# lh3/fermi

Measured on AMD Instinct MI355X. Metric: reads/sec through FMD backward-search (unitig overlap discovery), higher is better.
Workload: dtype u64

## Files before the change

### fermi_amd/csrc/fmd_kernel_common.h

```cpp
#pragma once
#include "fmd_internal.h"

#define NONE64 (~0ull)
#define FMD_SZ_MASK 0xffffffffffffull

__device__ __forceinline__ int comp6(int c) { return (c >= 1 && c <= 4) ? 5 - c : c; }

#include "fmd_search.h"

template <class T>
__device__ __forceinline__ T sel6(int c, T a0, T a1, T a2, T a3, T a4, T a5)
{
    T r = a0;
    r = c == 1 ? a1 : r; r = c == 2 ? a2 : r; r = c == 3 ? a3 : r; r = c == 4 ? a4 : r; r = c == 5 ? a5 : r;
    return r;
}

__device__ __forceinline__ void load_entry(const fmd_intv_t *e, uint64_t &x0, uint64_t &x1, uint64_t &sz, uint64_t &info)
{
    const uint4 *q = (const uint4 *)e;
    const uint4 a = q[0], b = q[1];
    x0 = (uint64_t)a.y << 32 | a.x; x1 = (uint64_t)a.w << 32 | a.z;
    sz = (uint64_t)b.y << 32 | b.x; info = (uint64_t)b.w << 32 | b.z;
}
__device__ __forceinline__ void store_entry(fmd_intv_t *e, uint64_t x0, uint64_t x1, uint64_t sz, uint64_t info)
{
    uint4 *q = (uint4 *)e;
    q[0] = make_uint4((uint32_t)x0, (uint32_t)(x0 >> 32), (uint32_t)x1, (uint32_t)(x1 >> 32));
    q[1] = make_uint4((uint32_t)sz, (uint32_t)(sz >> 32), (uint32_t)info, (uint32_t)(info >> 32));
}

#define FMD_CAND_NARROW 0x80000000u
struct FmdCand { uint64_t x0, x1, sz, D, r0; uint32_t depth; bool narrow; };
__device__ __forceinline__ FmdCand cand_decode(const uint4 a, const uint4 b)
{
    FmdCand c;
    c.narrow = (b.w & FMD_CAND_NARROW) != 0;
    c.x1 = (uint64_t)a.w << 32 | a.z;
    if (c.narrow) {
        c.x0 = (uint64_t)(a.y & 0xffu) << 32 | a.x; c.r0 = (uint64_t)((a.y >> 8) & 0xffu) << 32 | b.z; c.depth = a.y >> 16;
        c.sz = b.w & 63u; c.D = (uint64_t)b.y << 32 | b.x;
    } else {
        c.x0 = (uint64_t)a.y << 32 | a.x; c.sz = ((uint64_t)b.y << 32 | b.x) & 0xffffffffffffull; c.depth = b.z; c.D = 0; c.r0 = 0;
    }
    return c;
}
__device__ __forceinline__ void cand_store(fmd_intv_t *e, bool narrow, uint64_t x0, uint64_t x1, uint64_t sz, uint32_t depth, uint64_t D, uint64_t r0)
{
    uint4 *q = (uint4 *)e;
    const uint32_t x0h = (uint32_t)(x0 >> 32);
    q[0] = make_uint4((uint32_t)x0, narrow ? ((x0h & 0xffu) | ((uint32_t)(r0 >> 32) & 0xffu) << 8 | depth << 16) : x0h, (uint32_t)x1, (uint32_t)(x1 >> 32));
    q[1] = make_uint4(narrow ? (uint32_t)D : (uint32_t)sz, narrow ? (uint32_t)(D >> 32) : (uint32_t)(sz >> 32), narrow ? (uint32_t)r0 : depth,
                      narrow ? (FMD_CAND_NARROW | (uint32_t)sz) : 0u);
}

__device__ __forceinline__ uint64_t bits_below(int j) { return j >= 64 ? ~0ull : ((1ull << j) - 1); }

__device__ __forceinline__ uint4 grp_pick(const uint4 *img_k, int t_k, const uint4 *img_l, int t_l, uint32_t blk_k, uint32_t blk_l,
                                          bool has_k, bool has_l, uint32_t blk, uint32_t ch)
{
    const bool in_k = has_k && blk == blk_k, in_l = has_l && blk == blk_l;
    uint4 v = in_k ? img_k[(int)ch ^ t_k] : img_l[(int)ch ^ t_l];
    if (!in_k && !in_l) v = make_uint4(0, 0, 0, 0);
    return v;
}
__device__ __forceinline__ void grp_window(const uint4 *img_k, int t_k, const uint4 *img_l, int t_l, uint32_t blk_k, uint32_t blk_l,
                                           bool has_k, bool has_l, uint32_t blk_p, uint32_t off_p, uint4 &a, uint4 &b, uint4 &c)
{
    uint32_t blk = blk_p, ch = (off_p + 1) >> 5;
    if (ch >= FMD_BLK_CHUNKS) { ch -= FMD_BLK_OWN_CHUNKS; ++blk; }
    a = grp_pick(img_k, t_k, img_l, t_l, blk_k, blk_l, has_k, has_l, blk, ch);
    if (++ch == FMD_BLK_CHUNKS) { ch = FMD_BLK_CHUNKS - FMD_BLK_OWN_CHUNKS; ++blk; }
    b = grp_pick(img_k, t_k, img_l, t_l, blk_k, blk_l, has_k, has_l, blk, ch);
    if (++ch == FMD_BLK_CHUNKS) { ch = FMD_BLK_CHUNKS - FMD_BLK_OWN_CHUNKS; ++blk; }
    c = grp_pick(img_k, t_k, img_l, t_l, blk_k, blk_l, has_k, has_l, blk, ch);
}
__device__ __forceinline__ uint64_t win64(uint32_t w0, uint32_t w1, uint32_t w2, uint32_t sh)
{
    const uint32_t lo = __builtin_amdgcn_alignbit(w1, w0, sh), hi = __builtin_amdgcn_alignbit(w2, w1, sh);
    return (uint64_t)hi << 32 | lo;
}
template <class T>
__device__ __forceinline__ T win_before(T X, T Y, T Z, T cx, T cy, T cz)
{
    return ~(X | Y | Z) | (Z & ~X & (cx | cy)) | (X & Y & (cx ^ cy)) | (Y & ~X & cx & ~cy) | (X & ~Y & ~Z & cx & cz);
}
__device__ __forceinline__ uint64_t range64(uint32_t a, uint32_t b)
{
    return bits_below((int)b) & ~bits_below((int)a);
}


#define FMD_GRP_CLASSES 6
__device__ __host__ __forceinline__ constexpr int fmd_grp_size(int k) { return k == 0 ? 4 : k == 1 ? 8 : k == 2 ? 12 : k == 3 ? 16 : k == 4 ? 21 : 32; }
#define FMD_FAST_CHUNK 16
#define FMD_FAST_MAX_WAVES 8192
#define FMD_LIST_HOLE 0xffffffffu
#define FMD_LIST_RESUME 0x8000u
__device__ __forceinline__ void fmd_resume_encode(uint4 *e, uint64_t x1, uint32_t sz, uint64_t D, uint64_t r0, uint32_t pos, uint32_t round, uint32_t n_nei, uint32_t nei0, uint32_t lf,
                                                  uint32_t cat = 0, uint32_t flags8 = 0)
{
    e[0] = make_uint4((uint32_t)x1, ((uint32_t)(x1 >> 32) & 0xffu) | round << 8 | n_nei << 24, (uint32_t)D, (uint32_t)(D >> 32));
    e[1] = make_uint4((uint32_t)r0, ((uint32_t)(r0 >> 32) & 0xffu) | nei0 << 8, sz | pos << 16, (lf & 0x1ffffu) | cat << 17 | (flags8 & 0xffu) << 22);
}
__device__ __forceinline__ bool fmd_resume_fits(uint32_t round, uint32_t n_nei, uint32_t nei0, uint32_t pos) { return round < 65536u && n_nei < 256u && nei0 < 65536u && pos < 65536u; }
__device__ __forceinline__ void fmd_resume_decode(const uint4 a, const uint4 b, uint64_t &x1, uint32_t &sz, uint64_t &D, uint64_t &r0, uint32_t &pos, uint32_t &round, uint32_t &n_nei,
                                                  uint32_t &nei0, uint32_t &lf, uint32_t &cat, uint32_t &flags8)
{
    x1 = (uint64_t)(a.y & 0xffu) << 32 | a.x; round = (a.y >> 8) & 0xffffu; n_nei = a.y >> 24; D = (uint64_t)a.w << 32 | a.z;
    r0 = (uint64_t)(b.y & 0xffu) << 32 | b.x; nei0 = b.y >> 8; sz = b.z & 0xffffu; pos = b.z >> 16; lf = b.w & 0x1ffffu; cat = (b.w >> 17) & 31u; flags8 = (b.w >> 22) & 0xffu;
}
#define FMD_LANE_CHUNK 64
#define FMD_FAST_RESERVE (2 * FMD_FAST_MAX_WAVES * FMD_LANE_CHUNK)

#define FMD_CLS_CNT_STRIDE 32
#define FMD_CLS_HEADER_U32 640
#define FMD_CLS_LISTS (3 * FMD_GRP_CLASSES + 1)
#define FMD_CLS_SLOW FMD_GRP_CLASSES
static_assert(FMD_CLS_LISTS * FMD_CLS_CNT_STRIDE <= FMD_CLS_HEADER_U32, "one counter line per list");
__host__ __device__ __forceinline__ constexpr int fmd_cls_fast(int k) { return FMD_GRP_CLASSES + 1 + k; }
__host__ __device__ __forceinline__ constexpr int fmd_cls_cnt_off(int c) { return c * FMD_CLS_CNT_STRIDE; }
template <class P>
__host__ __device__ __forceinline__ constexpr P fmd_cls_list(P area, int c, size_t np)
{
    const size_t gl = 2 * np + 2 * (size_t)FMD_FAST_RESERVE;
    const P slow = area + FMD_CLS_HEADER_U32 + gl * FMD_GRP_CLASSES;
    if (c == FMD_CLS_SLOW) return slow;
    return c < FMD_CLS_SLOW ? area + FMD_CLS_HEADER_U32 + gl * c : slow + np + 2 * np * (size_t)(c - FMD_CLS_SLOW - 1);
}
template <class P> __host__ __device__ __forceinline__ constexpr P fmd_cls_late(P area, size_t np) { return fmd_cls_list(area, FMD_CLS_LISTS, np); }
template <class P> __host__ __device__ __forceinline__ constexpr P fmd_cls_fix(P area, size_t np) { return fmd_cls_late(area, np) + np; }
#define FMD_CLS_WORDS_PER_STRAND (6 * FMD_GRP_CLASSES + 3)
#define FMD_CLS_PART_U32 (FMD_CLS_HEADER_U32 + 2 * FMD_GRP_CLASSES * FMD_FAST_RESERVE)
__host__ __device__ __forceinline__ constexpr size_t fmd_cls_part_off(int part, size_t b) { return (size_t)part * FMD_CLS_PART_U32 + b * FMD_CLS_WORDS_PER_STRAND; }
static_assert(fmd_cls_fix<size_t>(0, 1000) + 1000 == fmd_cls_part_off(1, 1000) && fmd_cls_fix<size_t>(0, 1) + 1 == fmd_cls_part_off(1, 1), "a part's lists end where the next part begins");

enum FmdClsWord {
    FMD_CW_COUNT = 0,
    FMD_CW_DEAL = 16,
    FMD_CW_DOWN = 4,
    FMD_CW_DOWN_DEAL = FMD_CW_DOWN + FMD_CW_DEAL,
    FMD_CW_HANDED = 8,
    FMD_CW_HANDED_AT0 = 9,
    FMD_CW_FAST_ROUNDS = 10,
    FMD_CW_FAST_LIVE = 11,
    FMD_CW_FAST_HELD = 12,
    FMD_CW_FAST_ROUNDS2 = 13,
    FMD_CW_LATE = 4,
    FMD_CW_GRP_ROUNDS = 12,
    FMD_CW_GRP_LIVE = 13,
    FMD_CW_GRP_HELD = 14,
    FMD_CW_FIX = 20,
};
template <int... W> constexpr bool fmd_cw_distinct()
{
    const int w[] = {W...};
    for (size_t i = 0; i < sizeof...(W); ++i) {
        if (w[i] < 0 || w[i] >= FMD_CLS_CNT_STRIDE) return false;
        for (size_t j = 0; j < i; ++j) if (w[j] == w[i]) return false;
    }
    return true;
}
static_assert(fmd_cw_distinct<FMD_CW_COUNT, FMD_CW_DEAL>(), "a general list's counter line");
static_assert(fmd_cw_distinct<FMD_CW_COUNT, FMD_CW_DEAL, FMD_CW_DOWN, FMD_CW_DOWN_DEAL, FMD_CW_HANDED, FMD_CW_HANDED_AT0, FMD_CW_FAST_ROUNDS, FMD_CW_FAST_LIVE, FMD_CW_FAST_HELD,
                              FMD_CW_FAST_ROUNDS2>(), "a fast list's counter line");
static_assert(fmd_cw_distinct<FMD_CW_COUNT, FMD_CW_LATE, FMD_CW_GRP_ROUNDS, FMD_CW_GRP_LIVE, FMD_CW_GRP_HELD, FMD_CW_FIX>(), "the slow list's counter line");

struct FmdOvlClasses {
    uint32_t *cnt;
    uint32_t *lst[FMD_GRP_CLASSES];
    uint32_t *lslow;
    uint32_t *fast[2 * FMD_GRP_CLASSES];
};

__device__ __forceinline__ int fmd_ovl_list_of(uint32_t m, uint32_t len, bool w63, bool wnarrow, bool w32, int use_fast, int min_cls)
{
    int c = FMD_CLS_SLOW;
    if (w63 && len < 65535u) {
#pragma unroll
        for (int k = FMD_GRP_CLASSES - 1; k >= 0; --k) if (k >= min_cls && m <= (uint32_t)fmd_grp_size(k)) c = k;
        if (c < FMD_CLS_SLOW && wnarrow && use_fast) c += fmd_cls_fast(w32 ? FMD_GRP_CLASSES : 0);
    }
    return c;
}

#define FMD_WALK_SPLIT 32u
struct FmdWalkPark {
    unsigned long long k, x0, x1, sz;
    uint4 bases;
    uint4 pad;
};
static_assert(sizeof(FmdWalkPark) == 64, "one line per parked strand");
```

### fermi_amd/csrc/fmd_ovlp.hip

```cpp
#include <stdlib.h>
#include <string.h>
#include "fmd_ovlp_internal.h"

struct BatchLayout { size_t srev, listA, listB, cls, total; uint32_t stride_r, cap; };
static BatchLayout batch_layout(size_t n, uint32_t max_len, int min_match)
{
    BatchLayout L;
    const size_t stride_r = align_up((size_t)max_len, 16), cap = fmd_ovlp_list_cap(max_len, min_match);
    L.stride_r = (uint32_t)stride_r; L.cap = (uint32_t)cap;
    size_t o = 0;
    L.srev = o; o += align_up(n * stride_r, 256);
    L.listA = o; o += align_up(n * cap * sizeof(fmd_intv_t), 256);
    L.listB = o; o += align_up(n * cap * sizeof(fmd_intv_t), 256);
    L.cls = o; o += align_up(4 * fmd_cls_part_off(FMD_OVLP_MAX_PARTS, n), 256) + 256;
    L.total = o;
    return L;
}
extern "C" size_t fmd_ovlp_work_bytes(size_t n, uint32_t max_len, int min_match) { return batch_layout(n, max_len, min_match).total; }

struct OvlBatch {
    fmd_dev *h; FmdIndexView ix;
    const uint64_t *ids; int min_match; uint32_t max_len, max_nei, stride_r, cap, seq_stride;
    uint8_t *srev; fmd_intv_t *listA, *listB; uint32_t *cls;
    fmd_ovlp_rec_t *rec; fmd_intv_t *nei; uint8_t *seq;
    const uint32_t *gidx; FmdWalkPark *park;
    const uint32_t *keys;
    void carve(uint8_t *area, size_t n_area)
    {
        const BatchLayout L = batch_layout(n_area, max_len, min_match);
        stride_r = L.stride_r; cap = L.cap;
        srev = area + L.srev; listA = (fmd_intv_t *)(area + L.listA); listB = (fmd_intv_t *)(area + L.listB); cls = (uint32_t *)(area + L.cls);
    }
};

static bool ovl_tail2(const OvlBatch &o)
{
    const char *e = getenv("FMD_WALK_TAIL2");
    return o.gidx && fmd_walk_tail2_fits(o.stride_r, o.seq_stride) && !(e && atoi(e) == 0);
}
static bool ovl_tail2_cls(const OvlBatch &o)
{
    const char *e = getenv("FMD_WALK_CLS");
    return ovl_tail2(o) && !(e && atoi(e) == 0);
}
static int ovl_use_fast(void) { const char *ef = getenv("FMD_OVLP_FAST"); return fmd_nei_fast_available() && !(ef && atoi(ef) == 0); }
static int ovl_grp_down(void) { const char *e = getenv("FMD_GRP_DOWN"); return !(e && atoi(e) == 0); }
static int ovl_walk_phase(void) { const char *e = getenv("FMD_WALK_PHASE"); return !(e && atoi(e) == 0); }
static int ovl_min_cls(void) { const char *e = getenv("FMD_GRP4"); return e && atoi(e) == 0 ? 1 : 0; }

static void ovl_phase_a(const OvlBatch &o, hipStream_t st, size_t b, size_t np, int per_cu)
{
    WalkArgs a;
    a.ix = o.ix; a.n = np; a.min_match = o.min_match; a.stride_r = o.stride_r;
    a.listA = o.listA + b * (size_t)o.cap; a.cap = o.cap;
    uint8_t *srev = o.srev + b * (size_t)o.stride_r;
    if (!o.gidx) {
        a.ids = o.ids + b; a.rec = o.rec + b; a.srev = srev;
        fmd_launch_walk_whole(o.h, st, a, o.max_len, o.seq + b * (size_t)o.seq_stride, o.seq_stride, per_cu, 64);
        return;
    }
    a.rec = o.rec; a.park = o.park; a.gidx = o.gidx + b;
    if (!ovl_tail2(o)) {
        a.srev = srev;
        fmd_launch_walk_tail(o.h, st, a, o.max_len, o.seq, o.seq_stride, per_cu);
        return;
    }
    a.seq_out = o.seq; a.seq_stride = o.seq_stride; a.redo = (uint32_t *)srev;
    if (ovl_tail2_cls(o)) {
        a.cls = o.cls + fmd_cls_part_off(0, b); a.use_fast = ovl_use_fast(); a.min_cls = ovl_min_cls();
    }
    if (o.keys && ovl_walk_phase()) a.keys = o.keys + b;
    fmd_launch_walk_tail2(o.h, st, a, per_cu);
}

static int ovl_phase_b(const OvlBatch &o, hipStream_t st, size_t b, size_t np, int part, int per_cu, int fast_cu)
{
    NeiArgs a;
    a.ix = o.ix; a.n_cu = o.h->n_cu; a.grid = fmd_grid_for(o.h, np); a.np = np; a.min_match = o.min_match;
    a.srev = o.srev + b * (size_t)o.stride_r; a.stride_r = o.stride_r;
    a.listA = o.listA + b * (size_t)o.cap; a.listB = o.listB + b * (size_t)o.cap; a.cap = o.cap;
    a.gidx = o.gidx ? o.gidx + b : nullptr;
    a.rec = a.gidx ? o.rec : o.rec + b;
    a.nei = a.gidx ? o.nei : o.nei + b * (size_t)o.max_nei; a.max_nei = o.max_nei;
    a.seq = a.gidx ? o.seq : o.seq + b * (size_t)o.seq_stride; a.seq_stride = o.seq_stride;
    uint32_t *q2 = fmd_next_queue(o.h, st);
    uint32_t *cls = o.cls + fmd_cls_part_off(part, b);
    fmd_nei_lists_at(a, cls, np);
    const int use_fast = ovl_use_fast();
    if (!(part == 0 && ovl_tail2_cls(o))) {
        FMD_HIP_TRY(hipMemsetAsync(cls, 0, 4 * FMD_CLS_HEADER_U32, st));
        fmd_launch_classify(a, st, use_fast, ovl_min_cls());
    }
    bool side = false;
    FmdSideStream &slow = o.h->slow;
    if (slow.acquire(2)) {
        side = hipEventRecord(slow.ev[0], st) == hipSuccess && hipStreamWaitEvent(slow.stream, slow.ev[0], 0) == hipSuccess;
        if (!side) { (void)hipGetLastError(); slow.release(); }
    }
    {
        hipStream_t ss = side ? slow.stream : st;
        fmd_launch_nei_slow(a, ss, fmd_next_queue(o.h, ss), 0);
    }
    if (use_fast)
        for (int k = 0; k < 2 * FMD_GRP_CLASSES; ++k) {
            const int kg = k % FMD_GRP_CLASSES, wide = k >= FMD_GRP_CLASSES;
            if (fmd_nei_lane_enabled() && fmd_nei_lane_class_ok(kg, wide)) fmd_launch_nei_lane(a, kg, wide, fast_cu, st);
            else fmd_launch_nei_fast(a, kg, wide, fast_cu, st);
        }
    const uint32_t down_cap = ovl_grp_down() && np > 2 * (size_t)FMD_FAST_CHUNK ? (uint32_t)np : 0u;
    for (int k = 0; k < FMD_GRP_CLASSES; ++k) fmd_launch_nei_grp(a, k, per_cu, st, down_cap, 0);
    if (down_cap)
        for (int k = FMD_GRP_CLASSES - 2; k >= 0; --k) fmd_launch_nei_grp(a, k, per_cu, st, down_cap, 1);
    fmd_launch_nei_slow(a, st, q2, 1);
    fmd_launch_nei_fix(a, st, fmd_next_queue(o.h, st));
    if (side) {
        if (hipEventRecord(slow.ev[1], slow.stream) != hipSuccess || hipStreamWaitEvent(st, slow.ev[1], 0) != hipSuccess) { (void)hipGetLastError(); hipStreamSynchronize(slow.stream); }
        slow.release();
    }
    if (getenv("FMD_OVLP_STATS")) {
        uint32_t hs[FMD_CLS_HEADER_U32];
        hipStreamSynchronize(st);
        hipMemcpy(hs, cls, sizeof(hs), hipMemcpyDeviceToHost);
        const auto word = [&hs](int c, int w) { return hs[fmd_cls_cnt_off(c) + w]; };
        uint32_t nf = 0, nb = 0, ng = 0;
        for (int k = 0; k < 2 * FMD_GRP_CLASSES; ++k) { nf += word(fmd_cls_fast(k), FMD_CW_COUNT); nb += word(fmd_cls_fast(k), FMD_CW_HANDED); }
        for (int k = 0; k < FMD_GRP_CLASSES; ++k) ng += word(k, FMD_CW_COUNT);
        fprintf(stderr, "[M::fmd_ovlp] part of %zu strands: %u to the unforked path (%u of them handed on), %u slots of the general group kernels' lists (holes of the hand-over included), %u through the lane-per-strand kernel at once + %u handed back to it, %u fake forks fixed up\n",
                np, nf, nb, ng, word(FMD_CLS_SLOW, FMD_CW_COUNT), word(FMD_CLS_SLOW, FMD_CW_LATE), word(FMD_CLS_SLOW, FMD_CW_FIX));
        uint32_t ne[FMD_GRP_CLASSES];
        for (int k = 0; k < FMD_GRP_CLASSES; ++k) {
            const size_t slots = word(k, FMD_CW_COUNT);
            uint32_t *e = (uint32_t *)malloc(8 * slots + 8);
            ne[k] = 0;
            if (e && hipMemcpy(e, a.cl.lst[k], 8 * slots, hipMemcpyDeviceToHost) == hipSuccess)
                for (size_t i = 0; i < slots; ++i) ne[k] += e[2 * i] != FMD_LIST_HOLE;
            free(e);
        }
        static_assert(FMD_GRP_CLASSES == 6, "one %u per general class");
        fprintf(stderr, "[M::fmd_ovlp] ... of those slots %u %u %u %u %u %u hold a strand (general lists of the group classes, smallest first)\n", ne[0], ne[1], ne[2], ne[3], ne[4], ne[5]);
    }
#ifdef GRP_STATS
    {
        uint32_t hs[FMD_CLS_HEADER_U32];
        hipStreamSynchronize(st);
        hipMemcpy(hs, cls, sizeof(hs), hipMemcpyDeviceToHost);
        const auto word = [&hs](int c, int w) { return hs[fmd_cls_cnt_off(c) + w]; };
        const uint32_t gr = word(FMD_CLS_SLOW, FMD_CW_GRP_ROUNDS), gl = word(FMD_CLS_SLOW, FMD_CW_GRP_LIVE), gh = word(FMD_CLS_SLOW, FMD_CW_GRP_HELD);
        static_assert(FMD_GRP_CLASSES == 6, "one %u per general class");
        fprintf(stderr, "[grp stats] classes %u %u %u %u %u %u slow %u | wave rounds %u, live lanes %u (%.1f %%), lanes of groups holding a strand %u (%.1f %%)\n",
                word(0, FMD_CW_COUNT), word(1, FMD_CW_COUNT), word(2, FMD_CW_COUNT), word(3, FMD_CW_COUNT), word(4, FMD_CW_COUNT), word(5, FMD_CW_COUNT), word(FMD_CLS_SLOW, FMD_CW_COUNT),
                gr, gl, 100.0 * gl / (64.0 * gr), gh, 100.0 * gh / (64.0 * gr));
        for (int k = 0; k < 2 * FMD_GRP_CLASSES; ++k) {
            const int f = fmd_cls_fast(k);
            const uint32_t fr = word(f, FMD_CW_FAST_ROUNDS);
            if (word(f, FMD_CW_COUNT)) fprintf(stderr, "[fast stats] G=%d %s: %u strands, %u handed on (%u) | wave rounds %u (%u with a second base), live lanes %.1f %%, lanes of groups holding a strand %.1f %%\n",
                              fmd_grp_size(k % FMD_GRP_CLASSES), k >= FMD_GRP_CLASSES ? "64-bit" : "32-bit", word(f, FMD_CW_COUNT), word(f, FMD_CW_HANDED), word(f, FMD_CW_HANDED_AT0), fr,
                              word(f, FMD_CW_FAST_ROUNDS2), 100.0 * word(f, FMD_CW_FAST_LIVE) / (64.0 * fr), 100.0 * word(f, FMD_CW_FAST_HELD) / (64.0 * fr));
        }
    }
#endif
    return FMD_OK;
}

static void ovl_pipe_config(size_t n, int &parts, int &walk_cu, int &grp_cu, int &fast_cu)
{
    parts = 1; walk_cu = 8; grp_cu = 8; fast_cu = 8;
    const char *e = getenv("FMD_OVLP_PIPE");
    if (e) {
        int a = 0, b = 0, c = 0, d = 0;
        const int k = sscanf(e, "%d,%d,%d,%d", &a, &b, &c, &d);
        if (k >= 1 && a >= 1) parts = a < FMD_OVLP_MAX_PARTS ? a : FMD_OVLP_MAX_PARTS;
        if (k >= 2 && b >= 1) walk_cu = b;
        if (k >= 3 && c >= 1) grp_cu = c;
        if (k >= 4 && d >= 1) fast_cu = d;
    }
}
extern "C" int fmd_ovlp_dev(fmd_dev_t *h, void *stream_, size_t n, const uint64_t *d_ids, int min_match, uint32_t max_len,
                            uint32_t max_nei, fmd_ovlp_rec_t *d_rec, fmd_intv_t *d_nei, uint8_t *d_seq, uint32_t seq_stride,
                            void *d_work, size_t work_bytes)
{
    if (!h || (n && (!d_ids || !d_rec || !d_nei || !d_seq || !d_work)) || max_len == 0 || max_nei == 0 || min_match < 0) return FMD_E_ARG;
    if (n == 0) return FMD_OK;
    if (n >= 0xffffff00ull || work_bytes < fmd_ovlp_work_bytes(n, max_len, min_match)) return FMD_E_ARG;
    if (fmd_ovlp_list_cap(max_len, min_match) >= 4096) return FMD_E_ARG;
    FMD_HIP_TRY(hipSetDevice(h->device));
    hipStream_t st = (hipStream_t)stream_;
    OvlBatch o;
    o.h = h; o.ix = fmd_view(h);
    o.ids = d_ids; o.min_match = min_match; o.max_len = max_len; o.max_nei = max_nei; o.seq_stride = seq_stride;
    o.carve((uint8_t *)d_work, n);
    o.rec = d_rec; o.nei = d_nei; o.seq = d_seq; o.gidx = nullptr; o.park = nullptr; o.keys = nullptr;

    int parts, walk_cu, grp_cu, fast_cu;
    ovl_pipe_config(n, parts, walk_cu, grp_cu, fast_cu);
    if (parts > 1 && !h->aux.acquire(FMD_OVLP_MAX_PARTS + 1)) parts = 1;
    int rc = FMD_OK;
    if (parts == 1) {
        ovl_phase_a(o, st, 0, n, 0);
        rc = ovl_phase_b(o, st, 0, n, 0, 0, 0);
    } else {
        hipStream_t s2 = h->aux.stream;
        const size_t per = ((n + parts - 1) / parts + 63) & ~(size_t)63;
        int p = 0;
        bool join_ok = true;
        for (size_t b = 0; b < n && rc == FMD_OK; b += per, ++p) {
            const size_t np = n - b < per ? n - b : per;
            const bool last = b + per >= n;
            ovl_phase_a(o, st, b, np, p == 0 ? 0 : walk_cu);
            if (hipEventRecord(h->aux.ev[p], st) != hipSuccess || hipStreamWaitEvent(s2, h->aux.ev[p], 0) != hipSuccess) { join_ok = false; break; }
            rc = ovl_phase_b(o, s2, b, np, p, last ? 0 : grp_cu, last ? 0 : fast_cu);
        }
        if (!join_ok || hipEventRecord(h->aux.ev[FMD_OVLP_MAX_PARTS], s2) != hipSuccess ||
            hipStreamWaitEvent(st, h->aux.ev[FMD_OVLP_MAX_PARTS], 0) != hipSuccess) {
            hipStreamSynchronize(s2);
            if (!join_ok) { fmd_set_hip_error(hipGetLastError(), "overlap batch: event hand-over"); rc = FMD_E_HIP; }
        }
        h->aux.release();
    }
    if (rc != FMD_OK) return rc;
    FMD_CHECK_LAUNCH("overlap kernels");
    return FMD_OK;
}

struct SortedLayout { size_t park, keys_a, keys_b, vals_a, vals_b, tmp, tmp_bytes, batch_area, total; };
static SortedLayout sorted_layout(size_t n, size_t batch, uint32_t max_len, int min_match)
{
    SortedLayout L;
    size_t o = 0;
    L.park = o; o += align_up(n * sizeof(FmdWalkPark), 256);
    L.keys_a = o; o += align_up(n * 4, 256);
    L.keys_b = o; o += align_up(n * 4, 256);
    L.vals_a = o; o += align_up(n * 4, 256);
    L.vals_b = o; o += align_up(n * 4, 256);
    L.tmp_bytes = fmd_park_sort_temp_bytes(n);
    L.tmp = o; o += align_up(L.tmp_bytes, 256);
    L.batch_area = o;
    { const size_t ba = fmd_ovlp_work_bytes(batch, max_len, min_match), ad = align_up(n * 32, 256); o += ba > ad ? ba : ad; }
    L.total = o;
    return L;
}
extern "C" size_t fmd_ovlp_sorted_work_bytes(size_t n, size_t batch, uint32_t max_len, int min_match)
{
    if (batch == 0 || batch > n) batch = n;
    return sorted_layout(n, batch, max_len, min_match).total;
}
static bool sorted_eligible(const fmd_dev *h, size_t n, int min_match, uint32_t max_len)
{
    const char *e = getenv("FMD_OVLP_SORT");
    if (e && atoi(e) == 0) return false;
    return n < 0xffffff00ull && min_match >= (int)FMD_WALK_SPLIT && max_len >= FMD_WALK_SPLIT && h->ptab_d < (int)FMD_WALK_SPLIT;
}

extern "C" int fmd_ovlp_two_pass_ok(const fmd_dev_t *h, size_t n, int min_match, uint32_t max_len)
{
    return h && sorted_eligible(h, n, min_match, max_len) && fmd_ovlp_list_cap(max_len, min_match) < 4096 ? 1 : 0;
}
struct HeadLayout { size_t adm, keys_a, vals_a, tmp, tmp_bytes, total; };
static HeadLayout head_layout(size_t n)
{
    HeadLayout L;
    size_t o = 0;
    L.keys_a = o; o += align_up(n * 4, 256);
    L.vals_a = o; o += align_up(n * 4, 256);
    L.tmp_bytes = fmd_park_sort_temp_bytes(n);
    L.tmp = o; o += align_up(L.tmp_bytes, 256);
    L.adm = o; o += align_up(n * 32, 256);
    L.total = o;
    return L;
}
extern "C" size_t fmd_ovlp_head_work_bytes(size_t n) { return head_layout(n).total; }

extern "C" int fmd_ovlp_head_dev(fmd_dev_t *h, void *stream_, size_t n, const uint64_t *d_ids, int min_match, uint32_t max_len, fmd_ovlp_rec_t *d_rec,
                                 void *d_park, uint32_t *d_keys, uint32_t *d_order, void *d_work, size_t work_bytes)
{
    if (!h || (n && (!d_ids || !d_rec || !d_park || !d_keys || !d_order || !d_work)) || max_len == 0 || min_match < 0) return FMD_E_ARG;
    if (n == 0) return FMD_OK;
    if (!fmd_ovlp_two_pass_ok(h, n, min_match, max_len)) return FMD_E_ARG;
    const HeadLayout L = head_layout(n);
    if (work_bytes < L.total) return FMD_E_ARG;
    FMD_HIP_TRY(hipSetDevice(h->device));
    uint8_t *w = (uint8_t *)d_work;
    const int rc = fmd_ovlp_head(h, (hipStream_t)stream_, n, d_ids, min_match, d_rec, (FmdWalkPark *)d_park, (uint32_t *)(w + L.keys_a), (uint32_t *)(w + L.vals_a),
                            d_keys, d_order, w + L.tmp, L.tmp_bytes, (uint4 *)(w + L.adm));
    if (rc != FMD_OK) return rc;
    FMD_CHECK_LAUNCH("sorted overlap job: head");
    return FMD_OK;
}

static int ovl_tail(fmd_dev *h, hipStream_t st, size_t np, const uint32_t *rows, const uint32_t *keys, FmdWalkPark *park, const uint64_t *d_ids, int min_match, uint32_t max_len, uint32_t max_nei,
                    fmd_ovlp_rec_t *d_rec, fmd_intv_t *d_nei, uint8_t *d_seq, uint32_t seq_stride, uint8_t *area, size_t area_strands)
{
    OvlBatch o;
// ... 214 lines not shown
```

### fermi_amd/csrc/fmd_ovlp_lane.hip

```cpp
#include "fmd_ovlp_internal.h"

#define LANE_CHUNK FMD_LANE_CHUNK

template <typename M> struct LaneW;
template <> struct LaneW<uint32_t> {
    static constexpr uint32_t MAXW = 31;
    static __device__ __forceinline__ uint32_t below(uint32_t n) { return (1u << n) - 1u; }
    static __device__ __forceinline__ uint32_t popc(uint32_t v) { return (uint32_t)__popc(v); }
    static __device__ __forceinline__ int top(uint32_t v) { return 31 - __clz((int)v); }
};
template <> struct LaneW<uint64_t> {
    static constexpr uint32_t MAXW = 63;
    static __device__ __forceinline__ uint64_t below(uint32_t n) { return (1ull << n) - 1ull; }
    static __device__ __forceinline__ uint32_t popc(uint64_t v) { return (uint32_t)__popcll(v); }
    static __device__ __forceinline__ int top(uint64_t v) { return 63 - __clzll((long long)v); }
};

#define LC_PACK(r0, d, sz, pos) ((uint32_t)((r0) >> 32) & 0xffu) | (uint32_t)(d) << 8 | (uint32_t)(sz) << 14 | (uint32_t)(pos) << 20
#define LC_D(p) (((p) >> 8) & 63u)
#define LC_SZ(p) (((p) >> 14) & 63u)
#define LC_POS(p) ((p) >> 20)
#define LC_R0(p, lo) ((uint64_t)((p) & 0xffu) << 32 | (lo))
#define LANE_MAX_LEN 4095u


__device__ __forceinline__ void lane_flush_bases(uint8_t *seq_out, uint32_t seq_stride, uint32_t gs, uint32_t ori_l, uint32_t from, uint32_t to, uint64_t eb)
{
    uint8_t *row = seq_out + gs * (size_t)seq_stride;
    uint32_t p = ori_l + from, e = ori_l + to;
    if (e > seq_stride) e = seq_stride;
    while (p < e && (p & 3u)) { row[p] = (uint8_t)((eb & 3u) + 1u); eb >>= 2; ++p; }
    while (p + 4 <= e) {
        const uint32_t b = (uint32_t)eb & 0xffu;
        *(uint32_t *)(row + p) = ((b & 3u) | (b & 0xcu) << 6 | (b & 0x30u) << 12 | (b & 0xc0u) << 18) + 0x01010101u;
        eb >>= 8; p += 4;
    }
    while (p < e) { row[p] = (uint8_t)((eb & 3u) + 1u); eb >>= 2; ++p; }
}

#ifndef FMD_LANE_LB
#define FMD_LANE_LB 2
#endif

template <int G, typename M>
__global__ __launch_bounds__(64, FMD_LANE_LB) void k_ovl_nei_lane(FmdIndexView ix, const uint32_t *__restrict__ list, const uint32_t *__restrict__ list_n,
                                                                uint32_t cap, const fmd_intv_t *__restrict__ listA, fmd_intv_t *__restrict__ listB, fmd_ovlp_rec_t *__restrict__ rec,
                                                                fmd_intv_t *__restrict__ nei_out, uint32_t max_nei, uint8_t *__restrict__ seq_out, uint32_t seq_stride,
                                                                uint32_t *__restrict__ gen_list, uint32_t *__restrict__ gen_n, uint32_t *__restrict__ bail_n,
                                                                const uint32_t *__restrict__ gidx, uint32_t *__restrict__ queue, uint32_t tk_chunk, uint32_t slow_min, uint32_t adm_min)
{
    using W = LaneW<M>;
    constexpr bool WIDE = sizeof(M) == 8;
    __shared__ uint4 fmd_lds[WIDE ? FMD_WAVE_LDS_U4 : FMD_SLOT_U4];
    uint4 *lds = fmd_lds;
    const int lane = fmd_lane();
    const uint32_t N = *list_n;
    if (N == 0) return;
    FmdTickets tk;
    fmd_tickets_init(tk, queue, tk_chunk, N);

    bool active = false;
    uint32_t sid = 0, gs = 0, meta = 0, n_nei = 0, lf = 0, nei0 = 0, szw = 1, round = 0, am = 0;
    uint64_t X1 = 1;
    uint64_t eb = 0;
    uint32_t eb0 = 0;
    __shared__ uint4 cand[G * 64];
    uint4 *mc = cand + lane;
#define CD(e) (WIDE ? (M)((uint64_t)(e).y << 32 | (e).x) : (M)(e).x)
    uint32_t m_lane = 0;
    uint32_t res_cur = 0, res_end = 0, n_handed = 0;
    int hand = 0;
    bool slow = false;
    M sX = 0, sY = 0, sZ = 0;
    uint64_t sR0 = 0, sR1 = 0, sR2 = 0, sR3 = 0, sR4 = 0;
    int scs = 0;
    int st = 0;
    bool adm_bad = false;
    constexpr int HALVES = G > 8 ? 2 : 1, RAWN = (G + HALVES - 1) / HALVES;
    bool drained = false;

    for (;;) {
        {
            const uint64_t hm = __ballot(hand != 0);
            if (hm) {
                uint32_t meta_out = meta;
                if (hand == 2) {
                    const uint32_t mp = (uint32_t)__popc(am);
                    if (mp <= cap && fmd_resume_fits(round, n_nei, nei0, 0u)) {
                        for (uint32_t j = 0; j < m_lane; ++j)
                            if ((am >> j) & 1u) {
                                const uint4 e = mc[j * 64];
                                fmd_resume_encode((uint4 *)(listB + sid * (size_t)cap + __popc(am & ((1u << j) - 1u))), X1 + LC_D(e.w), LC_SZ(e.w), (uint64_t)CD(e),
                                                  LC_R0(e.w, e.z), LC_POS(e.w), round, n_nei, nei0, lf);
                            }
                        meta_out = mp | FMD_LIST_RESUME | (meta & 0xffff0000u);
                    }
                }
                const uint32_t n = (uint32_t)__popcll(hm), room = res_end - res_cur;
                uint32_t base = 0;
                if (room < n) {
                    if (lane == 0) { base = atomicAdd(gen_n, (uint32_t)LANE_CHUNK); atomicAdd(bail_n, n_handed); }
                    n_handed = 0;
                    base = (uint32_t)__builtin_amdgcn_readfirstlane((int)base);
                    gen_list[2 * (size_t)(base + lane)] = FMD_LIST_HOLE; gen_list[2 * (size_t)(base + lane) + 1] = 0;
                    asm volatile("s_waitcnt vmcnt(0)" ::: "memory");
                }
                if (hand) {
                    const uint32_t q = (uint32_t)fmd_below(hm), k = q < room ? res_cur + q : base + (q - room);
                    gen_list[2 * (size_t)k] = sid; gen_list[2 * (size_t)k + 1] = meta_out;
                    am = 0;
                }
                if (room < n) { res_cur = base + (n - room); res_end = base + LANE_CHUNK; }
                else res_cur += n;
                n_handed += n;
                hand = 0;
            }
        }
        uint4 raw[2 * RAWN];
        uint32_t l0 = 0, l1 = 0, g_in = 0;
        const uint64_t adm_wait_m = __ballot(st >= 2), adm_act_m = __ballot(active);
        const bool ld2 = st >= 2 && ((uint32_t)__popcll(adm_wait_m) >= adm_min || adm_act_m == 0);
        const uint32_t adm_m = meta & 0xffffu, adm_h0 = HALVES == 2 ? adm_m / 2 : 0u;
        const uint32_t adm_base = st == 2 ? adm_h0 : 0u, adm_cnt = st == 2 ? adm_m - adm_h0 : adm_h0;
        if (ld2) {
            const uint4 *q0 = (const uint4 *)(listA + sid * (size_t)cap + (cap - adm_m) + adm_base);
#pragma unroll
            for (int t = 0; t < RAWN; ++t) if ((uint32_t)t < adm_cnt) { raw[2 * t] = q0[2 * t]; raw[2 * t + 1] = q0[2 * t + 1]; }
            if (st == 2) g_in = gidx ? gidx[sid] : sid;
        }
        bool ld1 = false;
        {
            const bool want = st == 0 && !active && !drained && hand == 0;
            const size_t p = fmd_tickets_take(tk, queue, want, N);
            if (want && (p == (size_t)-1 || p >= N)) drained = true;
            else if (want) { l0 = list[2 * p]; l1 = list[2 * p + 1]; ld1 = true; }
        }
        const bool go = active && !slow;
        if (__ballot(go) == 0) fmd_fetch_wait();
        else {
            uint32_t bke, oke;
            fmd_split(X1 - 1, bke, oke);
            const uint4 *img_k, *img_l;
            int t_k, t_l;
            uint32_t ble = bke;
            bool sep = false;
            if (WIDE) {
                const FmdRank2 r = fmd_wave_rank2_fetch(ix, lds, go ? X1 - 1 : NONE64, go ? X1 - 1 + szw : NONE64);
                img_k = r.bk; img_l = r.bl; t_k = r.t; t_l = r.tl; ble = r.blk_l; sep = go && ble != bke;
            } else {
                fmd_fetch_slot<0>(ix, lds, bke, go);
                fmd_fetch_wait();
                img_k = img_l = lds + fmd_lds_base(lane, 0); t_k = t_l = fmd_chunk_xor(lane);
            }
            M X, Y, Z;
            {
                uint4 a, b, c;
                grp_window(img_k, t_k, img_l, t_l, bke, ble, true, sep, bke, oke, a, b, c);
                const uint32_t sh = (uint32_t)X1 & 31;
                if (WIDE) { X = (M)win64(a.x, b.x, c.x, sh); Y = (M)win64(a.y, b.y, c.y, sh); Z = (M)win64(a.z, b.z, c.z, sh); }
                else { X = (M)__builtin_amdgcn_alignbit(b.x, a.x, sh); Y = (M)__builtin_amdgcn_alignbit(b.y, a.y, sh); Z = (M)__builtin_amdgcn_alignbit(b.z, a.z, sh); }
            }
            const M mw = W::below(szw);
            const M any = (X | Y | Z) & mw, xa = X & any, ya = Y & any, za = Z & any;
            const M ends = ~(X | Y | Z) & mw;
            int cs = (xa ? 1 : 0) | (ya ? 2 : 0) | (za ? 4 : 0);
            const bool mixed = go && ((xa && xa != any) || (ya && ya != any) || (za && za != any) || cs > 4);
            uint64_t R[6] = {0, 0, 0, 0, 0, 0};
            if (__ballot(mixed)) { if (mixed) fmd_block_rank6<false>(img_k, t_k, oke + 1, R, bke); }
            if (!mixed) { uint64_t rz; const uint64_t rc = fmd_block_rank1z(img_k, t_k, oke + 1, cs, bke, rz); R[0] = rz; R[1] = R[2] = R[3] = R[4] = rc; }
            if (go) {
                if (!mixed && ends == 0) {
                    if (!(lf & 0x10000u)) lf = round + 1;
                    eb |= (uint64_t)(uint32_t)(4 - cs) << (2 * (round - eb0));
                    ++round;
                    if (round - eb0 == 32) { lane_flush_bases(seq_out, seq_stride, gs, meta >> 16, eb0, round, eb); eb = 0; eb0 = round; }
                    X1 = (cs == 1 ? ix.cnt[1] : cs == 2 ? ix.cnt[2] : cs == 3 ? ix.cnt[3] : ix.cnt[4]) + R[1];
                } else { slow = true; sX = X; sY = Y; sZ = Z; sR0 = R[0]; sR1 = R[1]; sR2 = R[2]; sR3 = R[3]; sR4 = R[4]; scs = cs | (mixed ? 8 : 0); }
            }
        }
        {
            const uint64_t sm = __ballot(slow);
            if (sm && ((uint32_t)__popcll(sm) >= slow_min || __ballot(active && !slow) == 0)) {
                if (slow) {
                    const M X = sX, Y = sY, Z = sZ;
                    int cs = scs & 7;
                    const bool mixed = (scs & 8) != 0;
                    const M mw = W::below(szw), any = (X | Y | Z) & mw, ends = ~(X | Y | Z) & mw;
                    const M m1 = X & ~Y & ~Z & mw, m2 = ~X & Y & ~Z & mw, m3 = X & Y & ~Z & mw, m4 = ~X & ~Y & Z & mw;
                    bool bail = false;
                    if (mixed) {
                        const M m5 = X & ~Y & Z & mw;
                        uint32_t u = 0;
                        for (uint32_t j = 0; j < m_lane; ++j) {
                            if ((am >> j) & 1u) {
                                const uint4 e = mc[j * 64];
                                const uint32_t d = LC_D(e.w), sz = LC_SZ(e.w);
                                const M mine = W::below(sz) << d;
                                const uint32_t nS = W::popc(ends & mine);
                                const uint32_t s1 = W::popc(m1 & mine), s2 = W::popc(m2 & mine), s3 = W::popc(m3 & mine), s4 = W::popc(m4 & mine), s5 = W::popc(m5 & mine);
                                const uint32_t o4 = nS, o3 = o4 + s4, o2 = o3 + s3, o1_ = o2 + s2, o5 = o1_ + s1;
                                const M D = CD(e);
                                if ((D >> o1_) & W::below(s1)) u |= 2u;
                                if ((D >> o2) & W::below(s2)) u |= 4u;
                                if ((D >> o3) & W::below(s3)) u |= 8u;
                                if ((D >> o4) & W::below(s4)) u |= 16u;
                                if ((D >> o5) & W::below(s5)) u |= 32u;
                            }
                        }
                        bail = __popc(u) >= 2 || (u & 32u);
                        cs = u ? __ffs((int)u) - 1 : 0;
                        if (cs > 4) cs = 0;
                    }
                    const uint64_t Rz = sR0, Rc = cs == 1 ? sR1 : cs == 2 ? sR2 : cs == 3 ? sR3 : cs == 4 ? sR4 : sR0;
                    const M Cw = !mixed ? any : cs == 1 ? m1 : cs == 2 ? m2 : cs == 3 ? m3 : cs == 4 ? m4 : (M)0;
                    slow = false;
                    const uint32_t ori_l = meta >> 16;
                    if (bail) { hand = 2; active = false; lane_flush_bases(seq_out, seq_stride, gs, ori_l, eb0, round, eb); }
                    else {
                    uint32_t nei_m = 0, child_m = 0;
                    for (uint32_t j = 0; j < m_lane; ++j) {
                        if ((am >> j) & 1u) {
                            const uint4 e = mc[j * 64];
                            const uint32_t d = LC_D(e.w), sz = LC_SZ(e.w);
                            const M mine = W::below(sz) << d, D = CD(e);
                            const uint32_t nS = W::popc(ends & mine);
                            uint32_t nc, coff;
                            if (mixed) {
                                const uint32_t s1 = W::popc(m1 & mine), s2 = W::popc(m2 & mine), s3 = W::popc(m3 & mine), s4 = W::popc(m4 & mine);
                                const uint32_t o4 = nS, o3 = o4 + s4, o2 = o3 + s3, o1_ = o2 + s2;
                                nc = cs == 1 ? s1 : cs == 2 ? s2 : cs == 3 ? s3 : cs == 4 ? s4 : 0u;
                                coff = cs == 1 ? o1_ : cs == 2 ? o2 : cs == 3 ? o3 : o4;
                            } else { nc = W::popc(any & mine); coff = sz - nc; }
                            if (round > 0 && nS == sz && D == W::below(sz)) nei_m |= 1u << j;
                            if ((D >> coff) & W::below(nc)) child_m |= 1u << j;
                        }
                    }
                    if (!(lf & 0x10000u)) lf = child_m ? round + 1 : (FMD_LFORK_ALL | 0x10000u);
                    const int f = nei_m ? __ffs((int)nei_m) - 1 : 32;
                    const uint32_t keep_m = f >= 32 ? child_m : child_m & ((1u << f) - 1u);
                    if (nei_m) {
                        const uint4 e = mc[f * 64];
                        const uint32_t d = LC_D(e.w), sz = LC_SZ(e.w), pos = LC_POS(e.w);
                        if (n_nei == 0) nei0 = ori_l - pos;
                        if (n_nei < max_nei)
                            store_entry(nei_out + gs * (size_t)max_nei + n_nei, LC_R0(e.w, e.z), ix.cnt[0] + Rz + W::popc(ends & W::below(d)), (uint64_t)sz, (uint64_t)(ori_l - pos));
                        ++n_nei;
                    }
                    if (n_nei > max_nei) {
                        rec[gs].flags |= FMD_OVLP_F_OVERFLOW;
                        active = false; am = 0;
                    } else if (keep_m) {
                        eb |= (uint64_t)(uint32_t)(4 - cs) << (2 * (round - eb0));
                        ++round;
                        if (round - eb0 == 32) { lane_flush_bases(seq_out, seq_stride, gs, ori_l, eb0, round, eb); eb = 0; eb0 = round; }
                        const int wl = 31 - __clz((int)keep_m);
                        uint32_t wb = 0, new_szw = 0;
                        for (int j = wl; j >= 0; --j) {
                            if ((keep_m >> j) & 1u) {
                                const uint4 e = mc[j * 64];
                                const uint32_t d = LC_D(e.w), sz = LC_SZ(e.w), pos = LC_POS(e.w);
                                const M mine = W::below(sz) << d, D = CD(e);
                                const uint32_t nS = W::popc(ends & mine);
                                uint32_t nc, coff;
                                if (mixed) {
                                    const uint32_t s1 = W::popc(m1 & mine), s2 = W::popc(m2 & mine), s3 = W::popc(m3 & mine), s4 = W::popc(m4 & mine);
                                    const uint32_t o4 = nS, o3 = o4 + s4, o2 = o3 + s3, o1_ = o2 + s2;
                                    nc = cs == 1 ? s1 : cs == 2 ? s2 : cs == 3 ? s3 : cs == 4 ? s4 : 0u;
                                    coff = cs == 1 ? o1_ : cs == 2 ? o2 : cs == 3 ? o3 : o4;
                                } else { nc = W::popc(any & mine); coff = sz - nc; }
                                const uint32_t before = W::popc(Cw & W::below(d));
                                if (j == wl) { wb = before; new_szw = nc; }
                                const uint64_t r0 = LC_R0(e.w, e.z) + W::popc(D & W::below(coff));
                                const M Dn = (D >> coff) & W::below(nc);
                                mc[j * 64] = make_uint4((uint32_t)Dn, WIDE ? (uint32_t)((uint64_t)Dn >> 32) : 0u, (uint32_t)r0, LC_PACK(r0, before - wb, nc, pos));
                            }
                        }
                        X1 = (cs == 1 ? ix.cnt[1] : cs == 2 ? ix.cnt[2] : cs == 3 ? ix.cnt[3] : ix.cnt[4]) + Rc + wb;
                        szw = new_szw;
                        am = keep_m;
                    } else {
                        lane_flush_bases(seq_out, seq_stride, gs, ori_l, eb0, round, eb);
                        fmd_ovlp_rec_t *o = rec + gs;
                        o->lfork = (uint16_t)(lf & 0xffffu);
                        o->rbeg = n_nei ? (int)(ori_l - nei0) : -1;
                        o->ext_len = n_nei > 1 ? 0 : (int)round;
                        o->n_nei = (int32_t)n_nei;
                        active = false; am = 0;
                    }
                    }
                }
            }
        }
        if (ld2) {
            const uint32_t m = adm_m, ori_l = meta >> 16;
            if (st == 2) {
                gs = g_in;
                round = 0; n_nei = 0; lf = 0; nei0 = 0; am = 0; eb = 0; eb0 = 0;
                adm_bad = m == 0 || m > (uint32_t)G || ori_l > LANE_MAX_LEN;
                uint64_t x1w = 1; uint32_t szw_ = 1;
#pragma unroll
                for (int t = 0; t < RAWN; ++t) if ((uint32_t)t + 1 == adm_cnt) { const FmdCand cw = cand_decode(raw[2 * t], raw[2 * t + 1]); x1w = cw.x1; szw_ = (uint32_t)cw.sz; }
                adm_bad |= szw_ > W::MAXW || szw_ == 0;
                X1 = x1w; szw = szw_;
                m_lane = adm_bad ? 0u : m;
            }
#pragma unroll
            for (int t = 0; t < RAWN; ++t)
                if ((uint32_t)t < adm_cnt && !adm_bad) {
                    const uint32_t j = adm_base + (uint32_t)t;
                    const FmdCand cd = cand_decode(raw[2 * t], raw[2 * t + 1]);
                    const uint64_t d = cd.x1 - X1;
                    adm_bad |= !cd.narrow || cd.x1 < X1 || d + cd.sz > szw || cd.sz == 0 || cd.depth > ori_l;
                    mc[j * 64] = make_uint4((uint32_t)cd.D, (uint32_t)(cd.D >> 32), (uint32_t)cd.r0, LC_PACK(cd.r0, d & 63u, cd.sz & 63u, (ori_l - cd.depth) & 0xfffu));
                    am |= 1u << j;
                }
            if (st == 2 && adm_h0 != 0 && !adm_bad) st = 3;
            else {
                if (adm_bad) { hand = 1; am = 0; }
                else active = true;
                st = 0;
            }
        }
        if (ld1) { sid = l0; meta = l1; st = 2; }
        asm volatile("s_waitcnt lgkmcnt(0)" ::: "memory");
        if (__ballot(active || st != 0 || hand != 0 || !drained) == 0) { if (lane == 0 && n_handed) atomicAdd(bail_n, n_handed); break; }
    }
}

static int lane_blocks_per_cu(const void *fn, size_t lds_bytes)
{
    return fmd_resident_per_cu(fn, lds_bytes, 20, "k_ovl_nei_lane");
}
int fmd_nei_lane_enabled(void)
{
    const char *e = getenv("FMD_NEI_LANE");
    return !(e && atoi(e) == 0);
}
int fmd_nei_lane_class_ok(int cls, int wide) { (void)wide; return cls >= 0 && cls <= 4; }

void fmd_launch_nei_lane(const NeiArgs &a, int cls, int wide, int per_cu_cap, hipStream_t st)
{
    const int fk = cls + (wide ? FMD_GRP_CLASSES : 0), fl = fmd_cls_fast(fk);
    uint32_t *queue = a.cnt(fl, FMD_CW_DEAL);
    const char *e = getenv("FMD_LANE_WAVES");
    const char *et = getenv("FMD_LANE_TICKETS");
    const uint32_t tk_chunk = et && atoi(et) >= 16 ? (uint32_t)atoi(et) : 256u;
    const char *es = getenv("FMD_LANE_BATCH");
    const uint32_t slow_min = es && atoi(es) >= 1 ? (uint32_t)atoi(es) : 32u;
    const char *ea = getenv("FMD_LANE_ADM_GATE");
    const uint32_t adm_min = ea && atoi(ea) >= 1 ? (uint32_t)atoi(ea) : 1u;
#define LANE_LAUNCH_(K, MM) do { \
        static int cached = 0; \
        if (!cached) cached = lane_blocks_per_cu((const void *)k_ovl_nei_lane<fmd_grp_size(K), MM>, sizeof(uint4) * ((sizeof(MM) == 8 ? FMD_WAVE_LDS_U4 : FMD_SLOT_U4) + 64 * fmd_grp_size(K))); \
        int per = cached; \
        if (per_cu_cap > 0 && per_cu_cap < per) per = per_cu_cap; \
        if (e && atoi(e) > 0 && atoi(e) < per) per = atoi(e); \
        int grid = a.n_cu * per; \
        if (grid > FMD_FAST_MAX_WAVES) grid = FMD_FAST_MAX_WAVES; \
        k_ovl_nei_lane<fmd_grp_size(K), MM><<<grid, 64, 0, st>>>(a.ix, a.cl.fast[fk], a.cnt(fl), a.cap, a.listA, a.listB, a.rec, a.nei, a.max_nei, a.seq, a.seq_stride, \
                                                                 a.cl.lst[cls], a.cnt(cls), a.cnt(fl, FMD_CW_HANDED), a.gidx, queue, tk_chunk, slow_min, adm_min); \
    } while (0)
#define LANE_LAUNCH2(K) do { if (wide) LANE_LAUNCH_(K, uint64_t); else LANE_LAUNCH_(K, uint32_t); } while (0)
    switch (cls) {
    case 0: LANE_LAUNCH2(0); break;
    case 1: LANE_LAUNCH2(1); break;
    case 2: LANE_LAUNCH2(2); break;
    case 3: LANE_LAUNCH2(3); break;
    default: LANE_LAUNCH2(4); break;
    }
#undef LANE_LAUNCH2
#undef LANE_LAUNCH_
}
```

Before: 266.7 million.

## Inline self-end rounds and fast-close simple strands in lane-per-strand kernel

Adds two inline shortcuts to the lane-per-strand neighbour kernel, both on by default through FMD_LANE_INLINE. First, a first-round self-end whose end count stays under the minimum leading depth is kept as a pending mask instead of forcing the lane into the slow path. The pending mask is applied lazily to the per-candidate entries only when they are needed. Second, strands whose closing round is trivially a single full-width neighbour skip the per-candidate loop. The aim is fewer divergent slow rounds and fewer LDS passes, at the cost of extra register state, more branches, and a template-instantiated stats variant.

New measurement: 273.8 million (median of 6 runs). +2.6%, better.

```diff
diff --git a/fermi_amd/csrc/fmd_kernel_common.h b/fermi_amd/csrc/fmd_kernel_common.h
--- a/fermi_amd/csrc/fmd_kernel_common.h
+++ b/fermi_amd/csrc/fmd_kernel_common.h
@@ -146,6 +146,12 @@
     FMD_CW_FAST_LIVE = 11,
     FMD_CW_FAST_HELD = 12,
     FMD_CW_FAST_ROUNDS2 = 13,
+    FMD_CW_LANE_ADM = 21,
+    FMD_CW_LANE_QUIET = 22,
+    FMD_CW_LANE_SELF = 23,
+    FMD_CW_LANE_CLOSE = 24,
+    FMD_CW_LANE_FULL = 25,
+    FMD_CW_LANE_MAT = 26,
     FMD_CW_LATE = 4,
     FMD_CW_GRP_ROUNDS = 12,
     FMD_CW_GRP_LIVE = 13,
@@ -163,7 +169,7 @@
 }
 static_assert(fmd_cw_distinct<FMD_CW_COUNT, FMD_CW_DEAL>(), "a general list's counter line");
 static_assert(fmd_cw_distinct<FMD_CW_COUNT, FMD_CW_DEAL, FMD_CW_DOWN, FMD_CW_DOWN_DEAL, FMD_CW_HANDED, FMD_CW_HANDED_AT0, FMD_CW_FAST_ROUNDS, FMD_CW_FAST_LIVE, FMD_CW_FAST_HELD,
-                              FMD_CW_FAST_ROUNDS2>(), "a fast list's counter line");
+                              FMD_CW_FAST_ROUNDS2, FMD_CW_LANE_ADM, FMD_CW_LANE_QUIET, FMD_CW_LANE_SELF, FMD_CW_LANE_CLOSE, FMD_CW_LANE_FULL, FMD_CW_LANE_MAT>(), "a fast list's counter line");
 static_assert(fmd_cw_distinct<FMD_CW_COUNT, FMD_CW_LATE, FMD_CW_GRP_ROUNDS, FMD_CW_GRP_LIVE, FMD_CW_GRP_HELD, FMD_CW_FIX>(), "the slow list's counter line");
 
 struct FmdOvlClasses {
diff --git a/fermi_amd/csrc/fmd_ovlp.hip b/fermi_amd/csrc/fmd_ovlp.hip
--- a/fermi_amd/csrc/fmd_ovlp.hip
+++ b/fermi_amd/csrc/fmd_ovlp.hip
@@ -138,6 +138,13 @@
         }
         static_assert(FMD_GRP_CLASSES == 6, "one %u per general class");
         fprintf(stderr, "[M::fmd_ovlp] ... of those slots %u %u %u %u %u %u hold a strand (general lists of the group classes, smallest first)\n", ne[0], ne[1], ne[2], ne[3], ne[4], ne[5]);
+        uint32_t ln[6] = {0, 0, 0, 0, 0, 0}, adm64 = 0;
+        for (int k = 0; k < 2 * FMD_GRP_CLASSES; ++k) {
+            for (int i = 0; i < 6; ++i) ln[i] += word(fmd_cls_fast(k), FMD_CW_LANE_ADM + i);
+            if (k >= FMD_GRP_CLASSES) adm64 += word(fmd_cls_fast(k), FMD_CW_LANE_ADM);
+        }
+        fprintf(stderr, "[M::fmd_ovlp] ... one lane per strand: %u strands admitted (%u with 64-bit masks), lane rounds: %u quiet, %u self-end inline, %u closing past the loops, %u through the loops of the full round (%u of them applied a pending self-end round first)\n",
+                ln[0], adm64, ln[1], ln[2], ln[3], ln[4], ln[5]);
     }
 #ifdef GRP_STATS
     {
diff --git a/fermi_amd/csrc/fmd_ovlp_lane.hip b/fermi_amd/csrc/fmd_ovlp_lane.hip
--- a/fermi_amd/csrc/fmd_ovlp_lane.hip
+++ b/fermi_amd/csrc/fmd_ovlp_lane.hip
@@ -42,12 +42,24 @@
 #define FMD_LANE_LB 2
 #endif
 
-template <int G, typename M>
+template <typename M>
+__device__ __forceinline__ void lane_self_end(M E0, M &D, uint32_t &w)
+{
+    using W = LaneW<M>;
+    const uint32_t d = LC_D(w), sz = LC_SZ(w);
+    const uint32_t nS0 = W::popc(E0 & (W::below(sz) << d));
+    D >>= nS0;
+    w = (w & 0xfff000ffu) | (d - W::popc(E0 & W::below(d))) << 8 | (sz - nS0) << 14;
+}
+
+struct LaneStats { uint32_t adm, quiet, self_end, closing, full, mat; };
+
+template <int G, typename M, bool STATS>
 __global__ __launch_bounds__(64, FMD_LANE_LB) void k_ovl_nei_lane(FmdIndexView ix, const uint32_t *__restrict__ list, const uint32_t *__restrict__ list_n,
                                                                 uint32_t cap, const fmd_intv_t *__restrict__ listA, fmd_intv_t *__restrict__ listB, fmd_ovlp_rec_t *__restrict__ rec,
                                                                 fmd_intv_t *__restrict__ nei_out, uint32_t max_nei, uint8_t *__restrict__ seq_out, uint32_t seq_stride,
                                                                 uint32_t *__restrict__ gen_list, uint32_t *__restrict__ gen_n, uint32_t *__restrict__ bail_n,
-                                                                const uint32_t *__restrict__ gidx, uint32_t *__restrict__ queue, uint32_t tk_chunk, uint32_t slow_min, uint32_t adm_min)
+                                                                const uint32_t *__restrict__ gidx, uint32_t *__restrict__ queue, uint32_t tk_chunk, uint32_t slow_min, uint32_t adm_min, uint32_t inl)
 {
     using W = LaneW<M>;
     constexpr bool WIDE = sizeof(M) == 8;
@@ -78,6 +90,9 @@
     bool adm_bad = false;
     constexpr int HALVES = G > 8 ? 2 : 1, RAWN = (G + HALVES - 1) / HALVES;
     bool drained = false;
+    uint32_t dmin = 0;
+    M E0 = 0;
+    LaneStats stats = {0, 0, 0, 0, 0, 0};
 
     for (;;) {
         {
@@ -169,7 +184,10 @@
             if (__ballot(mixed)) { if (mixed) fmd_block_rank6<false>(img_k, t_k, oke + 1, R, bke); }
             if (!mixed) { uint64_t rz; const uint64_t rc = fmd_block_rank1z(img_k, t_k, oke + 1, cs, bke, rz); R[0] = rz; R[1] = R[2] = R[3] = R[4] = rc; }
             if (go) {
-                if (!mixed && ends == 0) {
+                const bool self_end = (inl & 1u) && !mixed && ends != 0 && round == 0 && W::popc(ends) <= dmin;
+                if ((!mixed && ends == 0) || self_end) {
+                    if (STATS) { if (self_end) ++stats.self_end; else ++stats.quiet; }
+                    if (self_end) { E0 = ends; szw -= W::popc(ends); }
                     if (!(lf & 0x10000u)) lf = round + 1;
                     eb |= (uint64_t)(uint32_t)(4 - cs) << (2 * (round - eb0));
                     ++round;
@@ -182,6 +200,30 @@
             const uint64_t sm = __ballot(slow);
             if (sm && ((uint32_t)__popcll(sm) >= slow_min || __ballot(active && !slow) == 0)) {
                 if (slow) {
+                    bool simple = false;
+                    if ((inl & 2u) && scs < 8 && round > 0 && (am & 1u) && n_nei < max_nei) {
+                        const M mw = W::below(szw), any = (sX | sY | sZ) & mw, ends = ~(sX | sY | sZ) & mw;
+                        const uint4 e0 = mc[0], ew = mc[(31 - __clz((int)am)) * 64];
+                        M D0 = CD(e0);
+                        uint32_t w0 = e0.w;
+                        lane_self_end<M>(E0, D0, w0);
+                        const uint32_t sz0 = LC_SZ(w0), na = W::popc(any);
+                        simple = W::popc(ends & (W::below(sz0) << LC_D(w0))) == sz0 && D0 == W::below(sz0) &&
+                                 ((lf & 0x10000u) || (((CD(ew) >> W::popc(E0)) >> (szw - na)) & W::below(na)) != 0);
+                    }
+                    if (STATS) { if (simple) ++stats.closing; else ++stats.full; }
+                    if (E0 != 0 && !simple) {
+                        if (STATS) ++stats.mat;
+                        for (uint32_t j = 0; j < m_lane; ++j)
+                            if ((am >> j) & 1u) {
+                                const uint4 e = mc[j * 64];
+                                M D = CD(e);
+                                uint32_t w = e.w;
+                                lane_self_end<M>(E0, D, w);
+                                mc[j * 64] = make_uint4((uint32_t)D, WIDE ? (uint32_t)((uint64_t)D >> 32) : 0u, e.z, w);
+                            }
+                        E0 = 0;
+                    }
                     const M X = sX, Y = sY, Z = sZ;
                     int cs = scs & 7;
                     const bool mixed = (scs & 8) != 0;
@@ -217,8 +259,9 @@
                     const uint32_t ori_l = meta >> 16;
                     if (bail) { hand = 2; active = false; lane_flush_bases(seq_out, seq_stride, gs, ori_l, eb0, round, eb); }
                     else {
-                    uint32_t nei_m = 0, child_m = 0;
-                    for (uint32_t j = 0; j < m_lane; ++j) {
+                    uint32_t nei_m = simple ? 1u : 0u, child_m = nei_m;
+                    const uint32_t m_loop = simple ? 0u : m_lane;
+                    for (uint32_t j = 0; j < m_loop; ++j) {
                         if ((am >> j) & 1u) {
                             const uint4 e = mc[j * 64];
                             const uint32_t d = LC_D(e.w), sz = LC_SZ(e.w);
@@ -239,7 +282,8 @@
                     const int f = nei_m ? __ffs((int)nei_m) - 1 : 32;
                     const uint32_t keep_m = f >= 32 ? child_m : child_m & ((1u << f) - 1u);
                     if (nei_m) {
-                        const uint4 e = mc[f * 64];
+                        uint4 e = mc[f * 64];
+                        if (E0 != 0) { M D = CD(e); lane_self_end<M>(E0, D, e.w); }
                         const uint32_t d = LC_D(e.w), sz = LC_SZ(e.w), pos = LC_POS(e.w);
                         if (n_nei == 0) nei0 = ori_l - pos;
                         if (n_nei < max_nei)
@@ -285,7 +329,7 @@
                         o->rbeg = n_nei ? (int)(ori_l - nei0) : -1;
                         o->ext_len = n_nei > 1 ? 0 : (int)round;
                         o->n_nei = (int32_t)n_nei;
-                        active = false; am = 0;
+                        active = false; am = 0; E0 = 0;
                     }
                     }
                 }
@@ -295,7 +339,7 @@
             const uint32_t m = adm_m, ori_l = meta >> 16;
             if (st == 2) {
                 gs = g_in;
-                round = 0; n_nei = 0; lf = 0; nei0 = 0; am = 0; eb = 0; eb0 = 0;
+                round = 0; n_nei = 0; lf = 0; nei0 = 0; am = 0; eb = 0; eb0 = 0; E0 = 0; dmin = 63;
                 adm_bad = m == 0 || m > (uint32_t)G || ori_l > LANE_MAX_LEN;
                 uint64_t x1w = 1; uint32_t szw_ = 1;
 #pragma unroll
@@ -313,17 +357,25 @@
                     adm_bad |= !cd.narrow || cd.x1 < X1 || d + cd.sz > szw || cd.sz == 0 || cd.depth > ori_l;
                     mc[j * 64] = make_uint4((uint32_t)cd.D, (uint32_t)(cd.D >> 32), (uint32_t)cd.r0, LC_PACK(cd.r0, d & 63u, cd.sz & 63u, (ori_l - cd.depth) & 0xfffu));
                     am |= 1u << j;
+                    const uint32_t lead = cd.D != 0 && (cd.D >> cd.sz) == 0 ? (uint32_t)__ffsll((long long)cd.D) - 1u : 0u;
+                    dmin = lead < dmin ? lead : dmin;
                 }
             if (st == 2 && adm_h0 != 0 && !adm_bad) st = 3;
             else {
                 if (adm_bad) { hand = 1; am = 0; }
-                else active = true;
+                else { active = true; if (STATS) ++stats.adm; }
                 st = 0;
             }
         }
         if (ld1) { sid = l0; meta = l1; st = 2; }
         asm volatile("s_waitcnt lgkmcnt(0)" ::: "memory");
         if (__ballot(active || st != 0 || hand != 0 || !drained) == 0) { if (lane == 0 && n_handed) atomicAdd(bail_n, n_handed); break; }
+    }
+    if (STATS) {
+        uint32_t *c = bail_n + (FMD_CW_LANE_ADM - FMD_CW_HANDED);
+        const uint32_t v[6] = {stats.adm, stats.quiet, stats.self_end, stats.closing, stats.full, stats.mat};
+#pragma unroll
+        for (int i = 0; i < 6; ++i) if (v[i]) atomicAdd(c + i, v[i]);
     }
 }
 
@@ -349,16 +401,20 @@
     const uint32_t slow_min = es && atoi(es) >= 1 ? (uint32_t)atoi(es) : 32u;
     const char *ea = getenv("FMD_LANE_ADM_GATE");
     const uint32_t adm_min = ea && atoi(ea) >= 1 ? (uint32_t)atoi(ea) : 1u;
-#define LANE_LAUNCH_(K, MM) do { \
+    const char *ei = getenv("FMD_LANE_INLINE");
+    const uint32_t inl = ei ? (uint32_t)atoi(ei) & 3u : 3u;
+    const bool stats = getenv("FMD_OVLP_STATS") != nullptr;
+#define LANE_LAUNCH_(K, MM) do { if (stats) LANE_LAUNCH__(K, MM, true); else LANE_LAUNCH__(K, MM, false); } while (0)
+#define LANE_LAUNCH__(K, MM, ST) do { \
         static int cached = 0; \
-        if (!cached) cached = lane_blocks_per_cu((const void *)k_ovl_nei_lane<fmd_grp_size(K), MM>, sizeof(uint4) * ((sizeof(MM) == 8 ? FMD_WAVE_LDS_U4 : FMD_SLOT_U4) + 64 * fmd_grp_size(K))); \
+        if (!cached) cached = lane_blocks_per_cu((const void *)k_ovl_nei_lane<fmd_grp_size(K), MM, ST>, sizeof(uint4) * ((sizeof(MM) == 8 ? FMD_WAVE_LDS_U4 : FMD_SLOT_U4) + 64 * fmd_grp_size(K))); \
         int per = cached; \
         if (per_cu_cap > 0 && per_cu_cap < per) per = per_cu_cap; \
         if (e && atoi(e) > 0 && atoi(e) < per) per = atoi(e); \
         int grid = a.n_cu * per; \
         if (grid > FMD_FAST_MAX_WAVES) grid = FMD_FAST_MAX_WAVES; \
-        k_ovl_nei_lane<fmd_grp_size(K), MM><<<grid, 64, 0, st>>>(a.ix, a.cl.fast[fk], a.cnt(fl), a.cap, a.listA, a.listB, a.rec, a.nei, a.max_nei, a.seq, a.seq_stride, \
-                                                                 a.cl.lst[cls], a.cnt(cls), a.cnt(fl, FMD_CW_HANDED), a.gidx, queue, tk_chunk, slow_min, adm_min); \
+        k_ovl_nei_lane<fmd_grp_size(K), MM, ST><<<grid, 64, 0, st>>>(a.ix, a.cl.fast[fk], a.cnt(fl), a.cap, a.listA, a.listB, a.rec, a.nei, a.max_nei, a.seq, a.seq_stride, \
+                                                                 a.cl.lst[cls], a.cnt(cls), a.cnt(fl, FMD_CW_HANDED), a.gidx, queue, tk_chunk, slow_min, adm_min, inl); \
     } while (0)
 #define LANE_LAUNCH2(K) do { if (wide) LANE_LAUNCH_(K, uint64_t); else LANE_LAUNCH_(K, uint32_t); } while (0)
     switch (cls) {
@@ -369,5 +425,6 @@
     default: LANE_LAUNCH2(4); break;
     }
 #undef LANE_LAUNCH2
+#undef LANE_LAUNCH__
 #undef LANE_LAUNCH_
 }
```
